# Yunwei729/WACV2023-High-Resolution-Depth-Estimation-for-Panoramas-Through-Perspective-Map-Registrations

Measured on AMD Instinct MI355X. Metric: panoramas/sec (whole node), 2048×1024 × 20 tiles, at 1/2/4/8 MI355X, higher is better.
Workload: dtype f32; 1 GPU; C3/C4: 64 panoramas per GPU per step, 2048x1024 output, 20 tiles of 512x512 (5x4 layout), 512x256 baseline; global_batch=64, out=2048x1024, tiles=20x512x512, parallelism=dp1 (panorama sharding, no collective)

## Files before the change

wacv2023-high-resolution-depth-estimation-for-panoramas-through-perspective-map-registrations_amd/csrc/pf_ctx.hpp:

```cpp
#pragma once
#include "../../include/panofuse.h"
#include "pf_internal.hpp"

#include <cstdarg>
#include <cstdio>
#include <cstring>
#include <string>
#include <vector>

namespace pf {

struct DevBuf {
    void* p = nullptr;
    size_t bytes = 0;
    DevBuf() = default;
    DevBuf(const DevBuf&) = delete;
    DevBuf& operator=(const DevBuf&) = delete;
    ~DevBuf()
    {
        if (p) (void)hipFree(p);
    }
};

struct LevelCache {
// ... 231 lines not shown

inline int check_tile_range(pf_ctx* c, int t0, int t1)
{
    if (t0 < 0 || t1 > c->ntiles || t0 > t1)
        return fail(c, PF_EINVAL, "tile range [%d,%d) outside [0,%d)", t0, t1, c->ntiles);
    return PF_OK;
}

int prepare_levels(pf_ctx* c, int out_w, int out_h, float zr0, float zr1);
int prepare_registration(pf_ctx* c, float zr0, float zr1);
const int2* reg_sample_index(pf_ctx* c, int ew, int eh, int ec);
const float* reg_sample_kf(pf_ctx* c, int ew, int eh, int ec);
int check_reg_grids(pf_ctx* c, const int* active);
void grid_tables(const LevelDims& L, std::vector<GridCol>& cols, std::vector<GridRow>& rows);

inline int level_at(pf_ctx* c, int out_w, int out_h, float zr0, float zr1, int level,
                    const LevelDims** L)
{
    int rc;
    if ((rc = prepare_levels(c, out_w, out_h, zr0, zr1))) return rc;
    if (level < 0 || level >= c->lc.nlevels) return fail(c, PF_EINVAL, "bad level %d", level);
    *L = &c->lc.dims[level];
    return PF_OK;
}

struct PassPlan {
    int T = 1, nchunks = 1;
    int stages = 1;
    double cost = 0;
};

struct JresPlan {
    bool on = false;
    int nb = 0, core = 0, K = 0, rounds = 0;
    bool half = false;
};

inline int strip_halo(int T) { return (T + kJacobiCols - 1) / kJacobiCols * kJacobiCols; }

struct StripGeom {
    int Tp, V, nstrips;
};
inline StripGeom strip_geometry(int T, int w)
{
    const int Tp = strip_halo(T), V = 64 * kJacobiCols - 2 * Tp;
    return {Tp, V, (w + V - 1) / V};
}

int jacobi_tcap(const LevelDims& L);
std::vector<PassPlan> plan_level(pf_ctx* c, const LevelDims& L, int tcap, int batch, bool fast,
                                 int band_rows = 0);
PassPlan plan_band_pass(pf_ctx* c, const LevelDims& L, int T, int band_rows, bool fast);
JresPlan jres_plan(pf_ctx* c, const LevelDims& L, int batch, bool fast);

struct JacobiRun {
    int first;
    const float* emap;
    int ew, eh, ec;
    long long estride;
    const GridCol* cols;
    const GridRow* rows;
    const float* prev;
    long long pstride;
    const float* lnorm;
    float *a, *b;
    uint16_t* out;
    long long ostride;
// ... 32 lines not shown
```

wacv2023-high-resolution-depth-estimation-for-panoramas-through-perspective-map-registrations_amd/csrc/pf_fuse.hip:

```cpp
#include "pf_ctx.hpp"

#include <cstdlib>

using namespace pf;

int pf::seed_tables(pf_ctx* c, const LevelDims& L, int ew, int eh, int ec)
{
    if (seed_tables_match(c, L, ew, eh, ec)) return PF_OK;
    std::vector<int> ecol(L.w + 2), erow(L.h + 2);
    for (int xx = -1; xx <= L.w; xx++) {
        const float az = (float)((double)((float)xx / (float)(L.w - 1) * 2.0f) * PF_MYPI);
        ecol[xx + 1] = (int)((double)az / (PF_MYPI * 2) * (double)(float)(ew - 1)) * ec;
    }
    for (int yy = -1; yy <= L.h; yy++) {
        const float zen = (float)((double)((float)yy / (float)(L.h - 1)) * PF_MYPI);
        erow[yy + 1] = (int)((double)zen / PF_MYPI * (double)(float)(eh - 1)) * ew * ec;
    }
    int rc;
    if ((rc = upload(c, c->seed_ecol, ecol)) || (rc = upload(c, c->seed_erow, erow))) return rc;
    const int key[5] = {L.w, L.h, ew, eh, ec};
    memcpy(c->seed_key, key, sizeof(key));
    return PF_OK;
}

// ... 36 lines not shown

static bool show_plans()
{
    static const bool show = getenv("PF_JPLAN") != nullptr;
    return show;
}

void pf::show_sweeps_plan(const LevelDims& L, int batch)
{
    if (show_plans())
        fprintf(stderr, "jacobi plan %dx%d band %d iters %d batch %d sweeps\n", L.w, L.h,
                L.h1 - L.h0 + 1, L.iters, batch);
}

static float* run_jres(pf_ctx* c, const LevelDims& L, const JacobiRun& r, const JresPlan& jp)
{
    JresArgs A{};
    A.src_mode = r.first;
    if (r.first == 2) {
        if (!r.emap || !seed_tables_match(c, L, r.ew, r.eh, r.ec)) return nullptr;
        A.ecol = (const int*)c->seed_ecol.p;
        A.erow = (const int*)c->seed_erow.p;
    }
    const long long st = (long long)L.w * L.h;
    A.src = r.a; A.sstride = st;
    A.prev = r.prev; A.pstride = r.pstride;
    A.emap = r.emap; A.estride = r.estride;
    A.lnorm = r.lnorm; A.lstride = st;
    A.hcol = r.hcol;
    float* dst = r.first == 0 ? r.b : r.a;
    A.dst = dst; A.dstride = st;
    A.out = r.out; A.ostride = r.ostride;
    A.w = L.w; A.h = L.h; A.h0 = L.h0; A.h1 = L.h1; A.iters = L.iters; A.batch = r.batch;
    A.nb = jp.nb; A.core = jp.core; A.K = jp.K; A.half = jp.half ? 1 : 0;
    uint32_t* sync = (uint32_t*)c->jres_sync.p;
    A.xbuf = (float*)c->jres_x.p;
    A.ticket = sync;
    A.err = sync + 1;
    A.flags = sync + 2;
    A.err_host = c->jres_err_h;
    static const int dbg = getenv("PF_JRES_DBG") ? atoi(getenv("PF_JRES_DBG")) : 0;
    A.dbg = dbg;
    A.spin_log2 = 24;
    if (c->jres_fault) {
        A.dbg |= 16;
        A.spin_log2 = c->jres_fault;
        c->jres_fault = 0;
    }
    A.tbase = c->jres_tk;
    A.fbase = c->jres_fb;
    c->jres_tk += (uint32_t)(r.batch * jp.nb);
    c->jres_fb += (uint32_t)(jp.rounds + 1);
    if (show_plans())
        fprintf(stderr, "jacobi plan %dx%d band %d iters %d batch %d resident: nb %d core %d K %d rounds %d\n",
                L.w, L.h, L.h1 - L.h0 + 1, L.iters, r.batch, jp.nb, jp.core, jp.K, jp.rounds);
    launch_jres(c->stream, A);
    return dst;
}

float* pf::run_jacobi(pf_ctx* c, const LevelDims& L, const JacobiRun& r, int* npasses)
{
    if (r.jp && r.jp->on) {
        if (npasses) *npasses = 1;
        return run_jres(c, L, r, *r.jp);
    }
    static const bool slow = getenv("PF_JSLOW") != nullptr;
    const bool fast = r.hcol && !slow;
    const std::vector<PassPlan> plan = plan_level(c, L, jacobi_tcap(L), r.batch, fast);
    if (r.first == 2 && r.emap && !seed_tables_match(c, L, r.ew, r.eh, r.ec)) return nullptr;
    JacobiPass P = jacobi_pass(c, L, r);
    const int band_rows = L.h1 - L.h0 + 1;
    float* src = (r.first == 0) ? r.a : nullptr;
    float* dst = (r.first == 0) ? r.b : r.a;
    if (show_plans()) {
        fprintf(stderr, "jacobi plan %dx%d band %d iters %d batch %d %s C%d:", L.w, L.h,
                band_rows, L.iters, r.batch, fast ? "packed" : "general", kJacobiCols);
        for (const PassPlan& pp : plan)
            fprintf(stderr, " T%d/n%d%s", pp.T, pp.nchunks, pp.stages > 1 ? "p" : "");
        fprintf(stderr, "\n");
    }
    int pass = 0;
    for (const PassPlan& pp : plan) {
        const int T = pp.T;
        set_pass_shape(P, T, band_rows, pp.nchunks);
        P.src_mode = pass == 0 ? r.first : 0;
        P.src = src;
        P.dst = dst;
        P.out_mode = (pass + 1 == (int)plan.size() && r.out) ? 1 : 0;
// ... 384 lines not shown
```

wacv2023-high-resolution-depth-estimation-for-panoramas-through-perspective-map-registrations_amd/csrc/pf_internal.hpp:

```cpp
#pragma once

#include <hip/hip_runtime.h>
#include <cstdint>
#include <vector>

#include "../../include/panofuse.h"

#pragma clang fp contract(off)

#define PF_MYPI 3.14159265359
#define PF_NAN_MARKER 0x7FBADBADu
#define PF_MAX_COVER 40

namespace pf {

struct TileGeom {
    float middle[3], hedge[3], vedge[3], corner0[3];
    float mm, hl, vl, pad;
    int w, h, c;
    int pix_off;
    long long off;
};

struct TileBox {
// ... 135 lines not shown
    int y = (int)((double)zen / PF_MYPI * (double)(float)(h - 1));
    return ((long long)y * w + x) * c;
}

static constexpr int kJacobiCols = 2;

struct JacobiPass {
    const float* src; long long sstride;
    const float* prev; long long pstride;
    const float* emap; long long estride;
    int ew, eh, ec, src_mode;
    const int* ecol; const int* erow;
    const GridCol* cols; const GridRow* rows;
    const float* lnorm; long long lstride;
    float* dst; long long dstride;
    uint16_t* out; long long ostride;
    int out_mode;
    int w, h, h0, h1;
    int V, Tp, nstrips, nchunks, rows_per_chunk;
    int row_lo, row_hi;
    const float* hcol;
};

struct JresArgs {
    const float* src; long long sstride;
    const float* prev; long long pstride;
    const float* emap; long long estride;
    const int* ecol; const int* erow;
    const float* lnorm; long long lstride;
    const float* hcol;
    float* dst; long long dstride;
    uint16_t* out; long long ostride;
    int w, h, h0, h1, iters, batch, src_mode;
    int nb, core, K;
    int half;
    float* xbuf;
    uint32_t* flags;
    uint32_t* ticket;
    uint32_t* err;
    uint32_t* err_host;
    uint32_t tbase, fbase;
    int dbg;
    int spin_log2;
};
int jres_region_rows(int w, bool half = false);
int jres_threads();
int jres_blocks_per_cu(int w, bool half);
void launch_jres(hipStream_t s, const JresArgs& A);

void launch_tapmap(hipStream_t s, const TileGeom* geom, const TapBox* tb, int ntiles,
                   long long max_points, const GridCol* cols, const GridRow* rows, int32_t* map);
static constexpr int kAuditWords = 6;
void launch_layout_audit(hipStream_t s, const TileGeom* geom, const TileBox* box, int ntiles,
                         const GridCol* cols, const GridRow* rows, LevelDims L,
                         unsigned long long* ctr);
void launch_targets_patch(hipStream_t s, const TileGeom* geom, const TileBox* box,
                          const TapBox* tb, int ntiles, const int32_t* map, const float* tiles,
                          long long tstride, const float* coeffs, LevelDims L, float* lnorm,
                          long long lstride, int batch, const uint32_t* tmask = nullptr,
                          int nmw = 0, TileValid tv = TileValid{0, 0.0f, 0.0f});
struct TgtLevel {
    LevelDims L;
    const TileBox* box;
    const uint32_t* tmask;
    int nmw;
    const TapBox* tb;
    const int32_t* map;
// ... 257 lines not shown
```

wacv2023-high-resolution-depth-estimation-for-panoramas-through-perspective-map-registrations_amd/csrc/pf_jacobi.hip:

```cpp
#include "pf_internal.hpp"

#include <cstdlib>
#include <cstring>

#ifndef PF_JLAG_WAVES
#define PF_JLAG_WAVES 1
#endif
#ifndef PF_JPK_GROUP
#define PF_JPK_GROUP 3
#endif
#ifndef PF_JFILL
#define PF_JFILL -1
#endif
#ifndef PF_JDRAIN
#define PF_JDRAIN 1
#endif
#ifndef PF_JLAG_WAVES_FAST
#define PF_JLAG_WAVES_FAST 3
#endif
#ifndef PF_JPIPE_FILL
#define PF_JPIPE_FILL 3
#endif
#ifndef PF_JLAG_PF
#define PF_JLAG_PF 2
#endif
static_assert(6 % (PF_JLAG_PF + 1) == 0, "the 6-step unroll needs a load-buffer period dividing 6");

namespace pf {

namespace {

__device__ __forceinline__ float dpp_from_left(float v)
{
    return __int_as_float(__builtin_amdgcn_mov_dpp(__float_as_int(v), 0x138, 0xF, 0xF, true));
}
__device__ __forceinline__ float dpp_from_right(float v)
{
    return __int_as_float(__builtin_amdgcn_mov_dpp(__float_as_int(v), 0x130, 0xF, 0xF, true));
}

typedef float f2 __attribute__((ext_vector_type(2)));

struct Row {
    f2 v;
};

}

enum { SRC_BUF = 0, SRC_UPSAMPLE = 1, SRC_SEED = 2 };

__device__ __forceinline__ f2 pk_add_clamp01(f2 a, f2 b)
{
    f2 r;
    asm("v_pk_add_f32 %0, %1, %2 clamp" : "=v"(r) : "v"(a), "v"(b));
    return r;
}

__device__ __forceinline__ float add_scalar(float a, float b)
{
    float r;
    asm("v_add_f32 %0, %1, %2" : "=v"(r) : "v"(a), "v"(b));
    return r;
}
__device__ __forceinline__ float fmac_from_right(float acc, float x, float q)
{
    asm("v_fmac_f32_dpp %0, %1, %2 wave_shl:1 row_mask:0xf bank_mask:0xf bound_ctrl:0"
        : "+v"(acc) : "v"(x), "v"(q));
    return acc;
}
__device__ __forceinline__ float fma_scalar(float a, float b, float c)
{
    float r;
    asm("v_fma_f32 %0, %1, %2, %3" : "=v"(r) : "v"(a), "v"(b), "v"(c));
    return r;
}

template <int T, int SRC, bool OUT16, bool FAST>
struct JLag {
    static constexpr int C = kJacobiCols;
    static_assert(C == 2, "a lane's columns are one pair: Row, the vector loads and stores, the wrap");
    static constexpr int PF = PF_JLAG_PF, NB = PF_JLAG_PF + 1;
    static constexpr int R = (2 * T + 1 + 5) / 6 * 6, NG = R / 6;
    Row Lr[R];
    Row H[T][3];
    Row In[NB];
    Row Lin[NB];
    float hcol[C];
    float vq;
    const JacobiPass* P;
    int w, xs0, vlo, vhi, r0, r1, h0, h1;
    int colbase;
    int lo;
    int rlo, rhi;
    const float *src, *prev, *emap, *lnorm;
    float* dst;
    uint16_t* out;

    __device__ __forceinline__ Row load_row(const float* base_ptr, int k) const
    {
        Row r;
        int kc = k < rlo ? rlo : (k > rhi ? rhi : k);
        const float* rp = base_ptr + ((long long)kc * w + colbase);
        float2 q = *reinterpret_cast<const float2*>(rp + lo);
        r.v[0] = q.x; r.v[1] = q.y;
        return r;
    }

    __device__ __forceinline__ Row load_input(int k) const
    {
        if constexpr (SRC == SRC_BUF) {
            return load_row(src, k);
        } else {
            Row r;
#pragma unroll
            for (int j = 0; j < C; j += 2) {
                int xr = xs0 + j, Y = k;
                if (xr < 0) { xr += w; Y -= 1; }
                else if (xr >= w) { xr -= w; Y += 1; }
                float v0 = 0.0f, v1 = 0.0f;
                if (Y >= 0 && Y < P->h) {
                    if constexpr (SRC == SRC_UPSAMPLE) {
                        v0 = v1 = prev[(long long)(Y >> 1) * (w >> 1) + (xr >> 1)];
                    } else if (Y >= P->h0 && Y <= P->h1) {
                        const int ro = P->erow[Y + 1];
                        v0 = emap[ro + P->ecol[xr + 1]];
                        v1 = emap[ro + P->ecol[xr + 2]];
                    }
                }
                r.v[j] = v0;
                r.v[j + 1] = v1;
            }
            return r;
        }
    }

    static constexpr int slot(int ph, int a) { return ((ph - a) % 3 + 3) % 3; }

    template <int GB, int PH>
    __device__ __forceinline__ void ring_put(Row r)
    {
        if constexpr (FAST) {
#pragma unroll
            for (int j = 0; j < C; j++) r.v[j] = __builtin_isfinite(r.v[j]) ? r.v[j] : 0.0f;
        }
        Lr[((GB + PH) % R + R) % R] = r;
// ... 107 lines not shown
            f2 hh = f2{hcol[0], hcol[1]};
            if constexpr (ROWS) {
                const int row = k - 2 * t;
                const float hr = (row == h0 || row == h1) ? 0.0f : 1.0f;
                hh = hh * hr;
            }
            cur[g] = __builtin_elementwise_fma(Lv[g].v - cur[g], hh, H[t - 1][slot(PH, 2 * t)].v);
        }
#pragma unroll
        for (int g = 0; g < G; g++) {
            const int t = T0 + 1 + g;
            nw[t - 1].v = pk_add_clamp01(cur[g] * reg_, H[t - 1][slot(PH, 2 * t)].v * reg);
        }
    }
    template <int PH, int GB, int T0, bool ROWS, int NA, int LA = 1>
    __device__ __forceinline__ void sweep_packed(Row* nw, int k) const
    {
        constexpr int T1 = T0 + PF_JPK_GROUP < T ? T0 + PF_JPK_GROUP : T;
        if constexpr (T1 < T) sweep_packed<PH, GB, T1, ROWS, NA, LA>(nw, k);
        constexpr int TB = T1 < NA ? T1 : NA;
        constexpr int TA = T0 > LA - 1 ? T0 : LA - 1;
        if constexpr (TA < TB) {
            Row Lv[TB - TA];
            ring_get_range<GB, PH, TA + 1, TB>(Lv);
            sweep_packed_group<PH, TA, TB, ROWS>(Lv, nw, k);
        }
    }

    template <int PH, bool ROWS, int GB, int NA = T, int LA = 1>
    __device__ __forceinline__ void step(int k)
    {
        H[0][slot(PH, 1)] = In[(PH + NB - 1) % NB];
        ring_put<GB, PH>(Lin[PH % NB]);
        Lin[(PH + PF) % NB] = load_row(lnorm, k + PF);
        In[(PH + PF - 1) % NB] = load_input(k + PF - 1);
        Row nw[T];
        if constexpr (FAST) {
            sweep_packed<PH, GB, 0, ROWS, NA, LA>(nw, k);
        } else {
            static_assert(NA == T && LA == 1, "the general form has no fill / drain specialisation");
            Row Lv[T];
            ring_get_range<GB, PH, 1, T>(Lv);
            sweep_general<PH>(Lv, nw);
        }
#pragma unroll
        for (int t = 1; t < T; t++)
            if (t >= LA && t <= NA) H[t][slot(PH, 2 * t)] = nw[t - 1];
        if constexpr (NA < T) return;
        const int j = k - 2 * T;
        if (j >= r0 && j < r1 && xs0 >= vlo && xs0 < vhi) {
            const long long rowb = (long long)j * w + colbase;
            if constexpr (OUT16) {
                uint32_t qv[C];
#pragma unroll
                for (int p = 0; p < C; p++) qv[p] = (uint32_t)(nw[T - 1].v[p] * 65535.0f);
                *reinterpret_cast<uint32_t*>(out + rowb + lo) = qv[0] | (qv[1] << 16);
            } else {
                *reinterpret_cast<float2*>(dst + rowb + lo) = make_float2(nw[T - 1].v[0], nw[T - 1].v[1]);
            }
        }
    }

    template <bool ROWS, int G>
    __device__ __forceinline__ void group(int k)
    {
        step<0, ROWS, 6 * G>(k);
        step<1, ROWS, 6 * G>(k + 1);
// ... 91 lines not shown
        const bool dr = ND > 0 && gt >= NF + ND;
        if (!fill_from<ROWS, 0>(k, kend)) return;
        const int kd = dr ? k0 + 6 * (gt - ND) : kend;
        if (k < kd) {
            bool more = true;
            if constexpr (NF % NG != 0) more = groups_from<ROWS, NF % NG>(k, kd);
            while (more) more = groups_from<ROWS, 0>(k, kd);
        }
        if (dr) drain<ROWS>(__builtin_amdgcn_readfirstlane((gt - ND) % NG), k);
    }
};

template <int T, int SRC, bool OUT16, bool FAST>
__global__ void __launch_bounds__(256, FAST ? PF_JLAG_WAVES_FAST : PF_JLAG_WAVES)
k_jlag(JacobiPass P)
{
    using S_t = JLag<T, SRC, OUT16, FAST>;
    constexpr int C = S_t::C;
    const int lane = threadIdx.x & 63;
    const int wave = __builtin_amdgcn_readfirstlane(threadIdx.x >> 6);
    const int job = blockIdx.x * 4 + wave;
    if (job >= P.nstrips * P.nchunks) return;
    const int b = blockIdx.y;
    const int strip = job % P.nstrips, chunk = job / P.nstrips;
    S_t S;
    S.P = &P;
    S.w = P.w;
    S.h0 = P.h0;
    S.h1 = P.h1;
    S.colbase = strip * P.V - P.Tp;
    S.lo = lane * C;
    S.vq = -0.25f;
    asm volatile("" : "+v"(S.vq));
    S.rlo = P.h0;
    S.rhi = P.h1;
    S.xs0 = strip * P.V - P.Tp + lane * C;
    S.vlo = strip * P.V;
    S.vhi = min(S.vlo + P.V, P.w);
    S.r0 = P.row_lo + chunk * P.rows_per_chunk;
    S.r1 = min(S.r0 + P.rows_per_chunk, P.row_hi);
    S.src = P.src + b * P.sstride;
    S.prev = P.prev + b * P.pstride;
    S.emap = P.emap + b * P.estride;
    S.lnorm = P.lnorm + b * P.lstride;
    S.dst = P.dst + b * P.dstride;
    S.out = P.out + b * P.ostride;
#pragma unroll
    for (int j = 0; j < C; j++) S.hcol[j] = 0.0f;
    if constexpr (FAST) {
        if (S.xs0 >= 0 && S.xs0 < P.w)
#pragma unroll
            for (int j = 0; j < C; j++) S.hcol[j] = P.hcol[S.xs0 + j];
    }
#pragma unroll
    for (int t = 0; t < T; t++)
#pragma unroll
        for (int q = 0; q < 3; q++)
#pragma unroll
            for (int j = 0; j < C; j++) S.H[t][q].v[j] = 0.0f;
#pragma unroll
    for (int q = 0; q < S_t::NB; q++)
#pragma unroll
        for (int j = 0; j < C; j++) { S.In[q].v[j] = 0.0f; S.Lin[q].v[j] = 0.0f; }
#pragma unroll
    for (int q = 0; q < S_t::R; q++)
#pragma unroll
        for (int j = 0; j < C; j++) S.Lr[q].v[j] = 0.0f;
    const int k0 = S.r0 - T - 1;
    const int kend = S.r1 + 2 * T;
#pragma unroll
    for (int r = 0; r + 1 < S_t::PF; r++) S.In[r] = S.load_input(k0 + r);
#pragma unroll
    for (int r = 0; r < S_t::PF; r++) S.Lin[r] = S.load_row(S.lnorm, k0 + r);
    const int wlo = k0 - 2 * T, whi = kend + 3;
    const bool rows = (S.h0 >= wlo && S.h0 <= whi) || (S.h1 >= wlo && S.h1 <= whi);
    if (!FAST || rows) S.template run<true>(k0, kend);
    else S.template run<false>(k0, kend);
}

static constexpr int md(int a, int m) { return ((a % m) + m) % m; }

template <int TS, int S, int SI, int SRC, bool OUT16>
struct JPipe {
    static constexpr int C = kJacobiCols;
    static constexpr int T = TS * S;
    static constexpr int TB = SI * TS + 1, TE = TB + TS - 1;
    static constexpr int PF = PF_JLAG_PF, NB = PF_JLAG_PF + 1;
    static constexpr int R = (2 * TS + 1 + 5) / 6 * 6;
    static constexpr int NG = R / 6;
    static constexpr int G = PF_JPK_GROUP;
    Row H[TS][3];
    Row In[NB];
    Row Lin[NB];
    float* lring;
    const float* xin;
    float* xout;
    int lane_c;
    float hcol[C];
    float vq;
    const JacobiPass* P;
    int w, xs0, vlo, vhi, r0, r1, h0, h1, colbase, lo, rlo, rhi;
    const float *src, *prev, *emap, *lnorm;
    float* dst;
    uint16_t* out;

    __device__ __forceinline__ Row load_row(const float* base_ptr, int k) const
    {
        Row r;
        int kc = k < rlo ? rlo : (k > rhi ? rhi : k);
        const float2 q = *reinterpret_cast<const float2*>(base_ptr + ((long long)kc * w + colbase) + lo);
        r.v[0] = q.x; r.v[1] = q.y;
        return r;
    }
    __device__ __forceinline__ Row load_input(int k) const
    {
        if constexpr (SRC == SRC_BUF) {
            return load_row(src, k);
        } else {
            Row r;
            int xr = xs0, Y = k;
            if (xr < 0) { xr += w; Y -= 1; }
            else if (xr >= w) { xr -= w; Y += 1; }
            float v0 = 0.0f, v1 = 0.0f;
            if (Y >= 0 && Y < P->h) {
                if constexpr (SRC == SRC_UPSAMPLE) {
                    v0 = v1 = prev[(long long)(Y >> 1) * (w >> 1) + (xr >> 1)];
                } else if (Y >= P->h0 && Y <= P->h1) {
                    const int ro = P->erow[Y + 1];
                    v0 = emap[ro + P->ecol[xr + 1]];
                    v1 = emap[ro + P->ecol[xr + 2]];
                }
            }
            r.v[0] = v0;
            r.v[1] = v1;
            return r;
        }
    }
    __device__ __forceinline__ void lds_put(float* p, Row r) const
    {
        r.v[0] = __builtin_isfinite(r.v[0]) ? r.v[0] : 0.0f;
        r.v[1] = __builtin_isfinite(r.v[1]) ? r.v[1] : 0.0f;
        *reinterpret_cast<float2*>(p) = make_float2(r.v[0], r.v[1]);
    }
    __device__ __forceinline__ Row lds_get(const float* p) const
    {
        Row r;
        const float2 q = *reinterpret_cast<const float2*>(p);
        r.v[0] = q.x; r.v[1] = q.y;
        return r;
    }

    template <int PH, int T0, int T1, bool ROWS>
// ... 37 lines not shown
                const float hr = (row == h0 || row == h1) ? 0.0f : 1.0f;
                hh = hh * hr;
            }
            cur[g] = __builtin_elementwise_fma(Lv[t - TB].v - cur[g], hh, H[l][md(PH - 2 * t, 3)].v);
        }
#pragma unroll
        for (int g = 0; g < NGR; g++) {
            const int t = T0 + 1 + g, l = t - TB;
            nw[t - TB].v = pk_add_clamp01(cur[g] * reg_, H[l][md(PH - 2 * t, 3)].v * reg);
        }
    }
    template <int PH, int T0, bool ROWS, int NA>
    __device__ __forceinline__ void sweep(const Row* Lv, Row* nw, int k) const
    {
        constexpr int T1 = T0 + G < TE ? T0 + G : TE;
        constexpr int TB_ = T1 < NA ? T1 : NA;
        if constexpr (T0 < TB_) sweep_group<PH, T0, TB_, ROWS>(Lv, nw, k);
        if constexpr (T1 < TE) sweep<PH, T1, ROWS, NA>(Lv, nw, k);
    }

    template <int PH, bool ROWS, int GB, int NA = T>
    __device__ __forceinline__ void step(int k)
    {
        if constexpr (SI == 0) {
            H[0][md(PH - 1, 3)] = In[md(PH - 1, NB)];
        } else {
            H[0][md(PH - 2 * TB + 1, 3)] = lds_get(xin + md(PH - 1, 2) * (64 * C) + lane_c);
        }
        constexpr int QO = -2 * TB + 2;
        lds_put(lring + md(GB + PH + QO, R) * (64 * C) + lane_c, Lin[md(PH + QO, NB)]);
        Row Lv[TS];
#pragma unroll
        for (int t = TB; t <= TE; t++) Lv[t - TB] = lds_get(lring + md(GB + PH - 2 * t, R) * (64 * C) + lane_c);
        Lin[md(PH + QO + PF, NB)] = load_row(lnorm, k + QO + PF);
        if constexpr (SI == 0) In[md(PH + PF - 1, NB)] = load_input(k + PF - 1);
        Row nw[TS];
        sweep<PH, TB - 1, ROWS, NA>(Lv, nw, k);
#pragma unroll
        for (int t = TB; t < TE; t++)
            if (t <= NA) H[t - TB + 1][md(PH - 2 * t, 3)] = nw[t - TB];
        if constexpr (SI < S - 1) {
            if constexpr (TE <= NA)
                *reinterpret_cast<float2*>(xout + md(PH, 2) * (64 * C) + lane_c) =
                    make_float2(nw[TS - 1].v[0], nw[TS - 1].v[1]);
        } else if constexpr (NA == T) {
            const int j = k - 2 * T;
            if (j >= r0 && j < r1 && xs0 >= vlo && xs0 < vhi) {
                const long long rowb = (long long)j * w + colbase;
                if constexpr (OUT16) {
                    const uint32_t q0 = (uint32_t)(nw[TS - 1].v[0] * 65535.0f);
                    const uint32_t q1 = (uint32_t)(nw[TS - 1].v[1] * 65535.0f);
                    *reinterpret_cast<uint32_t*>(out + rowb + lo) = q0 | (q1 << 16);
                } else {
                    *reinterpret_cast<float2*>(dst + rowb + lo) =
                        make_float2(nw[TS - 1].v[0], nw[TS - 1].v[1]);
                }
            }
        }
        __syncthreads();
    }

    template <bool ROWS, int GI>
    __device__ __forceinline__ void group(int k)
    {
        step<0, ROWS, 6 * GI>(k);
        step<1, ROWS, 6 * GI>(k + 1);
        step<2, ROWS, 6 * GI>(k + 2);
// ... 34 lines not shown
            return fill_from<ROWS, F + 1>(k, kend);
        } else {
            return true;
        }
    }
    template <bool ROWS>
    __device__ __forceinline__ void run(int k0, int kend)
    {
        int k = k0;
        bool more = fill_from<ROWS, 0>(k, kend);
        if constexpr (NF % NG != 0) {
            if (more) more = groups_from<ROWS, NF % NG>(k, kend);
        }
        while (more) more = groups_from<ROWS, 0>(k, kend);
    }
};

template <int TS, int S, int SI, int SRC, bool OUT16>
__device__ __forceinline__ void jpipe_stage(const JacobiPass& P, int lane, int b, int strip,
                                            int chunk, float* lring, float* xchg)
{
    using S_t = JPipe<TS, S, SI, SRC, OUT16>;
    constexpr int T = S_t::T, C = S_t::C;
    S_t St;
    St.P = &P;
    St.w = P.w;
    St.h0 = P.h0;
    St.h1 = P.h1;
    St.colbase = strip * P.V - P.Tp;
    St.lo = lane * C;
    St.lane_c = lane * C;
    St.vq = -0.25f;
    asm volatile("" : "+v"(St.vq));
    St.rlo = P.h0;
    St.rhi = P.h1;
    St.xs0 = strip * P.V - P.Tp + lane * C;
    St.vlo = strip * P.V;
    St.vhi = min(St.vlo + P.V, P.w);
    St.r0 = P.row_lo + chunk * P.rows_per_chunk;
    St.r1 = min(St.r0 + P.rows_per_chunk, P.row_hi);
    St.src = P.src + b * P.sstride;
    St.prev = P.prev + b * P.pstride;
    St.emap = P.emap + b * P.estride;
    St.lnorm = P.lnorm + b * P.lstride;
    St.dst = P.dst + b * P.dstride;
    St.out = P.out + b * P.ostride;
    St.lring = lring + SI * (S_t::R * 64 * C);
    St.xin = SI > 0 ? xchg + (SI - 1) * (2 * 64 * C) : nullptr;
    St.xout = SI < S - 1 ? xchg + SI * (2 * 64 * C) : nullptr;
    St.hcol[0] = St.hcol[1] = 0.0f;
    if (St.xs0 >= 0 && St.xs0 < P.w) { St.hcol[0] = P.hcol[St.xs0]; St.hcol[1] = P.hcol[St.xs0 + 1]; }
#pragma unroll
    for (int l = 0; l < TS; l++)
#pragma unroll
        for (int q = 0; q < 3; q++) St.H[l][q].v = f2{0.0f, 0.0f};
#pragma unroll
    for (int q = 0; q < S_t::NB; q++) { St.In[q].v = f2{0.0f, 0.0f}; St.Lin[q].v = f2{0.0f, 0.0f}; }
    const int k0 = St.r0 - T - 1;
    const int kend = St.r1 + 2 * T;
    constexpr int QO = -2 * S_t::TB + 2;
    if constexpr (SI == 0) {
#pragma unroll
        for (int r = 0; r + 1 < S_t::PF; r++) St.In[md(r, S_t::NB)] = St.load_input(k0 + r);
    }
#pragma unroll
    for (int r = 0; r < S_t::PF; r++) St.Lin[md(QO + r, S_t::NB)] = St.load_row(St.lnorm, k0 + QO + r);
    const int wlo = k0 - 2 * T, whi = kend + 3;
    const bool rows = (St.h0 >= wlo && St.h0 <= whi) || (St.h1 >= wlo && St.h1 <= whi);
    if (rows) St.template run<true>(k0, kend);
    else St.template run<false>(k0, kend);
}

template <int TS, int S, int SRC, bool OUT16>
__global__ void __launch_bounds__(64 * S) k_jpipe(JacobiPass P)
{
    constexpr int C = kJacobiCols, R = JPipe<TS, S, 0, SRC, OUT16>::R;
    const int lane = threadIdx.x & 63;
    const int wave = __builtin_amdgcn_readfirstlane(threadIdx.x >> 6);
    const int job = blockIdx.x;
    if (job >= P.nstrips * P.nchunks) return;
    const int b = blockIdx.y;
    const int strip = job % P.nstrips, chunk = job / P.nstrips;
    __shared__ float lring[S * R * 64 * C];
    __shared__ float xchg[(S > 1 ? S - 1 : 1) * 2 * 64 * C];
    for (int i = threadIdx.x; i < (S > 1 ? S - 1 : 1) * 2 * 64 * C; i += 64 * S) xchg[i] = 0.0f;
    __syncthreads();
    if (wave == 0) jpipe_stage<TS, S, 0, SRC, OUT16>(P, lane, b, strip, chunk, lring, xchg);
    if constexpr (S > 1) { if (wave == 1) jpipe_stage<TS, S, (S > 1 ? 1 : 0), SRC, OUT16>(P, lane, b, strip, chunk, lring, xchg); }
    if constexpr (S > 2) { if (wave == 2) jpipe_stage<TS, S, (S > 2 ? 2 : 0), SRC, OUT16>(P, lane, b, strip, chunk, lring, xchg); }
    if constexpr (S > 3) { if (wave == 3) jpipe_stage<TS, S, (S > 3 ? 3 : 0), SRC, OUT16>(P, lane, b, strip, chunk, lring, xchg); }
}

#if !defined(PF_JPART) || PF_JPART == 0
__global__ void __launch_bounds__(256) k_border(const float* __restrict__ prev, long long pstride,
                                                LevelDims L, float* __restrict__ a,
                                                float* __restrict__ bb, long long stride,
                                                uint16_t* __restrict__ out, long long ostride)
{
    const int top = L.h0 * L.w;
// ... 214 lines not shown
```

wacv2023-high-resolution-depth-estimation-for-panoramas-through-perspective-map-registrations_amd/csrc/pf_jres.hip:

```cpp
#include "pf_internal.hpp"

namespace pf {

namespace {

typedef float f2 __attribute__((ext_vector_type(2)));
typedef uint32_t u4v __attribute__((ext_vector_type(4)));

__device__ __forceinline__ float dpp_shr(float v)
{
    return __int_as_float(__builtin_amdgcn_mov_dpp(__float_as_int(v), 0x138, 0xF, 0xF, true));
}
__device__ __forceinline__ float dpp_rol(float v)
{
    return __int_as_float(__builtin_amdgcn_mov_dpp(__float_as_int(v), 0x134, 0xF, 0xF, false));
}
__device__ __forceinline__ float fmac_rol(float acc, float x, float q)
{
    asm("s_nop 1\n\tv_fmac_f32_dpp %0, %1, %2 wave_rol:1 row_mask:0xf bank_mask:0xf"
        : "+v"(acc) : "v"(x), "v"(q));
    return acc;
}
__device__ __forceinline__ f2 pk_add_clamp01(f2 a, f2 b)
{
// ... 91 lines not shown
        f2 up[NP], dn[NP], s1[NP], n[NP];
#pragma unroll
        for (int k = 0; k < NP; k++) {
            up[k] = up_lds ? up_lds[64 * k] : f2{0.0f, 0.0f};
            dn[k] = dn_lds ? dn_lds[64 * k] : f2{0.0f, 0.0f};
            s1[k] = b[RS > 1 ? 1 : 0][k];
            n[k] = b[0][k];
        }
        if constexpr (RS > 1) rows_mid<1, HAS_EDGE>(n, dn, em);
        if (HAS_EDGE && (em & 1u)) row<0, true>(up, RS > 1 ? s1 : dn);
        else row<0, false>(up, RS > 1 ? s1 : dn);
    }
};

template <int CPL, int RS, int NWV, int SRC, bool OUT16>
__global__ void __launch_bounds__(64 * NWV) k_jres(JresArgs A)
{
    using S_t = JRes<CPL, RS, NWV, SRC, OUT16>;
    constexpr int NP = S_t::NP, NW = S_t::NW;
    __shared__ f2 lds_edge[2][2][NW][NP][64];
    __shared__ uint32_t lds_ticket;
    const int tid = threadIdx.x;
    S_t S;
    S.lane = tid & 63;
    S.wv = __builtin_amdgcn_readfirstlane(tid >> 6);
    S.vq = -0.25f;
    asm volatile("" : "+v"(S.vq));
    const int lane = S.lane, wv = S.wv;
    if (tid == 0) lds_ticket = __hip_atomic_fetch_add(A.ticket, 1u, __ATOMIC_RELAXED, __HIP_MEMORY_SCOPE_AGENT);
    __syncthreads();
    const uint32_t t = __builtin_amdgcn_readfirstlane(lds_ticket - A.tbase);
    const int p = (int)(t / (uint32_t)A.nb), j = (int)(t % (uint32_t)A.nb);
    const int w = A.w;
    const int c0 = A.h0 + j * A.core;
    const int c1 = min(c0 + A.core, A.h1 + 1);
    const int K = A.K;
    const int rs = j == 0 ? A.h0 : c0 - K;
    const int re = j == A.nb - 1 ? A.h1 + 1 : min(c1 + K, A.h1 + 1);
    const int x0 = lane * CPL;
    const int qc0 = c0 - rs, qc1 = c1 - rs;

    {
        const float* lp = A.lnorm + p * A.lstride;
#pragma unroll
        for (int k = 0; k < NP; k++) {
            S.hc[k].x = A.hcol[x0 + 2 * k];
            S.hc[k].y = A.hcol[x0 + 2 * k + 1];
        }
#pragma unroll
        for (int r = 0; r < RS; r++) {
            const int Y = rs + wv * RS + r;
            const bool live = Y < re;
#pragma unroll
            for (int k = 0; k < NP; k++) {
                float v0 = 0.0f, v1 = 0.0f, l0 = 0.0f, l1 = 0.0f;
                if (live) {
                    const int x = x0 + 2 * k;
                    if constexpr (SRC == 2) {
                        const float* ep = A.emap + p * A.estride + A.erow[Y + 1];
                        v0 = ep[A.ecol[x + 1]];
                        v1 = ep[A.ecol[x + 2]];
                    } else if constexpr (SRC == 1) {
                        v0 = v1 = A.prev[p * A.pstride + (long long)(Y >> 1) * (w >> 1) + (x >> 1)];
                    } else {
                        const float2 q = *reinterpret_cast<const float2*>(A.src + p * A.sstride + (long long)Y * w + x);
                        v0 = q.x;
                        v1 = q.y;
                    }
// ... 211 lines not shown
```

wacv2023-high-resolution-depth-estimation-for-panoramas-through-perspective-map-registrations_amd/csrc/pf_plan.hip:

```cpp
#include "pf_ctx.hpp"

#include <cstdlib>

using namespace pf;

static int plan_simds(const pf_ctx* c)
{
    const int n = (int)(4.0 * c->num_cu * c->jacobi_share + 0.5);
    return n < 4 ? 4 : n;
}

struct JacobiTuning {
    int Tmax = 10;
    double step_overhead = 3.0, lone_cycles = 4.0;
    double pipe_overhead = 1.0;
    double launch_cost = 300.0;
};

static const JacobiTuning& jacobi_tuning()
{
    static const JacobiTuning tune = [] {
        JacobiTuning t;
        if (const char* e = getenv("PF_JT")) t.Tmax = atoi(e);
        if (const char* e = getenv("PF_JOVH")) t.step_overhead = atof(e);
// ... 81 lines not shown
    for (int r = L.iters; r > 0; r -= choice[r]) plan.push_back(opt[choice[r]]);
    if (c->jacobi_share < 1.0)
        for (PassPlan& pp : plan)
            if (pp.stages == 1)
                pp.nchunks = best_chunks(pp.T, band_rows, L.w, batch,
                                         jstream_waves_per_cu(pp.T, fast) / 4, plan_simds(c))
                                 .nchunks;
    char key[32];
    snprintf(key, sizeof(key), "PF_JN%d", L.w);
    if (const char* e = getenv(key))
        for (PassPlan& pp : plan) pp.nchunks = atoi(e) > 0 ? atoi(e) : pp.nchunks;
    return plan;
}

int pf::jacobi_tcap(const LevelDims& L)
{
    int cap = jacobi_tuning().Tmax;
    char key[32];
    snprintf(key, sizeof(key), "PF_JT%d", L.w);
    if (const char* e = getenv(key)) cap = atoi(e) > 0 ? atoi(e) : cap;
    if (L.h0 - 1 < cap) cap = L.h0 - 1;
    if (L.h - 2 - L.h1 < cap) cap = L.h - 2 - L.h1;
    while (cap >= 1) {
        int Tp = (cap + 3) / 4 * 4;
        if (128 - Tp <= L.w && L.w % 2 == 0) break;
        cap--;
    }
    return cap;
}

PassPlan pf::plan_band_pass(pf_ctx* c, const LevelDims& L, int T, int band_rows, bool fast)
{
    return best_chunks(T, band_rows, L.w, 1, jstream_waves_per_cu(T, fast) / 4, plan_simds(c));
}

JresPlan pf::jres_plan(pf_ctx* c, const LevelDims& L, int batch, bool fast)
{
    JresPlan jp;
    static const char* env = getenv("PF_JRES");
    const int mode = c->jres_mode >= 0 ? c->jres_mode : (env && atoi(env) == 0 ? 0 : 1);
    if (mode == 0 || !fast || batch < 1) return jp;
    const int rows = jres_region_rows(L.w);
    if (rows <= 0 || L.iters < 1) return jp;
    static int bpc_w[2][2] = {{-1, -1}, {-1, -1}};
    const int wi = L.w == 256 ? 0 : 1;
    const int band = L.h1 - L.h0 + 1;
    static const double xcost = getenv("PF_JRES_X") ? atof(getenv("PF_JRES_X")) : 2.5;
    static const int nb_env = getenv("PF_JRES_NB") ? atoi(getenv("PF_JRES_NB")) : 0;
    const int nb_force = c->jres_nb > 0 ? c->jres_nb : nb_env;
    static const double hcost = getenv("PF_JRES_HALFCOST") ? atof(getenv("PF_JRES_HALFCOST")) : 0.6;
    double best = 1e300;
    for (int hv = 0; hv < 2; hv++) {
        const int rows_h = hv ? jres_region_rows(L.w, true) : rows;
        if (rows_h <= 0) continue;
        if (bpc_w[wi][hv] < 0) bpc_w[wi][hv] = jres_blocks_per_cu(L.w, hv == 1);
        const int bpc = bpc_w[wi][hv];
        if (bpc < 1) continue;
        const double sweep = hv ? hcost : 1.0;
        for (int nb = 1; nb <= band && nb <= 64; nb++) {
            if (nb_force > 0 && nb != nb_force) continue;
            const int core = (band + nb - 1) / nb;
            if ((band + core - 1) / core != nb) continue;
            int K;
            if (nb == 1) {
                if (core > rows_h) continue;
                K = L.iters;
            } else {
                K = (rows_h - core) / 2;
                if (K > core) K = core;
                if (K > L.iters) K = L.iters;
                if (K < 1) continue;
            }
            const int rounds = (L.iters + K - 1) / K;
            const long long resident = (long long)c->num_cu * bpc;
            const long long waves = ((long long)batch * nb + resident - 1) / resident;
            const double cost = (double)waves * (L.iters * sweep + (rounds - 1) * xcost);
            if (cost < best) {
                best = cost;
                jp.on = true;
                jp.nb = nb;
                jp.core = core;
                jp.K = K;
                jp.rounds = rounds;
                jp.half = hv == 1;
            }
        }
    }
    return jp;
}
```

Baseline: 18160 panoramas/s.

## Use asymmetric edge/interior block cores in resident Jacobi and tighten row clamp windows

The resident Jacobi planner now lets edge blocks own a larger core (rows minus one halo) than interior blocks (rows minus two halos). It picks K from the register-resident row capacity, which should allow a larger K and fewer exchange rounds for the same block count. The streaming Jacobi kernels also clamp input and lnorm row loads to a per-chunk window widened by the halo rather than the whole band, which limits out-of-window reads. Risks are off-by-one errors in the block bounds and in the clamping, which could change numerics at chunk edges.

```diff
diff --git a/wacv2023-high-resolution-depth-estimation-for-panoramas-through-perspective-map-registrations_amd/csrc/pf_ctx.hpp b/wacv2023-high-resolution-depth-estimation-for-panoramas-through-perspective-map-registrations_amd/csrc/pf_ctx.hpp
--- a/wacv2023-high-resolution-depth-estimation-for-panoramas-through-perspective-map-registrations_amd/csrc/pf_ctx.hpp
+++ b/wacv2023-high-resolution-depth-estimation-for-panoramas-through-perspective-map-registrations_amd/csrc/pf_ctx.hpp
@@ -287,7 +287,7 @@
 
 struct JresPlan {
     bool on = false;
-    int nb = 0, core = 0, K = 0, rounds = 0;
+    int nb = 0, core_e = 0, core_i = 0, K = 0, rounds = 0;
     bool half = false;
 };
 
diff --git a/wacv2023-high-resolution-depth-estimation-for-panoramas-through-perspective-map-registrations_amd/csrc/pf_fuse.hip b/wacv2023-high-resolution-depth-estimation-for-panoramas-through-perspective-map-registrations_amd/csrc/pf_fuse.hip
--- a/wacv2023-high-resolution-depth-estimation-for-panoramas-through-perspective-map-registrations_amd/csrc/pf_fuse.hip
+++ b/wacv2023-high-resolution-depth-estimation-for-panoramas-through-perspective-map-registrations_amd/csrc/pf_fuse.hip
@@ -92,7 +92,7 @@
     A.dst = dst; A.dstride = st;
     A.out = r.out; A.ostride = r.ostride;
     A.w = L.w; A.h = L.h; A.h0 = L.h0; A.h1 = L.h1; A.iters = L.iters; A.batch = r.batch;
-    A.nb = jp.nb; A.core = jp.core; A.K = jp.K; A.half = jp.half ? 1 : 0;
+    A.nb = jp.nb; A.core_e = jp.core_e; A.core_i = jp.core_i; A.K = jp.K; A.half = jp.half ? 1 : 0;
     uint32_t* sync = (uint32_t*)c->jres_sync.p;
     A.xbuf = (float*)c->jres_x.p;
     A.ticket = sync;
@@ -112,8 +112,9 @@
     c->jres_tk += (uint32_t)(r.batch * jp.nb);
     c->jres_fb += (uint32_t)(jp.rounds + 1);
     if (show_plans())
-        fprintf(stderr, "jacobi plan %dx%d band %d iters %d batch %d resident: nb %d core %d K %d rounds %d\n",
-                L.w, L.h, L.h1 - L.h0 + 1, L.iters, r.batch, jp.nb, jp.core, jp.K, jp.rounds);
+        fprintf(stderr, "jacobi plan %dx%d band %d iters %d batch %d resident: nb %d core %d/%d K %d rounds %d\n",
+                L.w, L.h, L.h1 - L.h0 + 1, L.iters, r.batch, jp.nb, jp.core_e, jp.core_i, jp.K,
+                jp.rounds);
     launch_jres(c->stream, A);
     return dst;
 }
diff --git a/wacv2023-high-resolution-depth-estimation-for-panoramas-through-perspective-map-registrations_amd/csrc/pf_internal.hpp b/wacv2023-high-resolution-depth-estimation-for-panoramas-through-perspective-map-registrations_amd/csrc/pf_internal.hpp
--- a/wacv2023-high-resolution-depth-estimation-for-panoramas-through-perspective-map-registrations_amd/csrc/pf_internal.hpp
+++ b/wacv2023-high-resolution-depth-estimation-for-panoramas-through-perspective-map-registrations_amd/csrc/pf_internal.hpp
@@ -191,7 +191,7 @@
     float* dst; long long dstride;
     uint16_t* out; long long ostride;
     int w, h, h0, h1, iters, batch, src_mode;
-    int nb, core, K;
+    int nb, core_e, core_i, K;
     int half;
     float* xbuf;
     uint32_t* flags;
diff --git a/wacv2023-high-resolution-depth-estimation-for-panoramas-through-perspective-map-registrations_amd/csrc/pf_jacobi.hip b/wacv2023-high-resolution-depth-estimation-for-panoramas-through-perspective-map-registrations_amd/csrc/pf_jacobi.hip
--- a/wacv2023-high-resolution-depth-estimation-for-panoramas-through-perspective-map-registrations_amd/csrc/pf_jacobi.hip
+++ b/wacv2023-high-resolution-depth-estimation-for-panoramas-through-perspective-map-registrations_amd/csrc/pf_jacobi.hip
@@ -45,6 +45,12 @@
     f2 v;
 };
 
+__device__ __forceinline__ void row_window(int r0, int r1, int d, int h0, int h1, int& lo, int& hi)
+{
+    lo = min(max(r0 - d, h0), h1);
+    hi = max(min(r1 + d - 1, h1), lo);
+}
+
 }
 
 enum { SRC_BUF = 0, SRC_UPSAMPLE = 1, SRC_SEED = 2 };
@@ -91,12 +97,12 @@
     int w, xs0, vlo, vhi, r0, r1, h0, h1;
     int colbase;
     int lo;
-    int rlo, rhi;
+    int ilo, ihi, llo, lhi;
     const float *src, *prev, *emap, *lnorm;
     float* dst;
     uint16_t* out;
 
-    __device__ __forceinline__ Row load_row(const float* base_ptr, int k) const
+    __device__ __forceinline__ Row load_row(const float* base_ptr, int k, int rlo, int rhi) const
     {
         Row r;
         int kc = k < rlo ? rlo : (k > rhi ? rhi : k);
@@ -109,8 +115,9 @@
     __device__ __forceinline__ Row load_input(int k) const
     {
         if constexpr (SRC == SRC_BUF) {
-            return load_row(src, k);
+            return load_row(src, k, ilo, ihi);
         } else {
+            k = k < ilo ? ilo : (k > ihi ? ihi : k);
             Row r;
 #pragma unroll
             for (int j = 0; j < C; j += 2) {
@@ -284,7 +291,7 @@
     {
         H[0][slot(PH, 1)] = In[(PH + NB - 1) % NB];
         ring_put<GB, PH>(Lin[PH % NB]);
-        Lin[(PH + PF) % NB] = load_row(lnorm, k + PF);
+        Lin[(PH + PF) % NB] = load_row(lnorm, k + PF, llo, lhi);
         In[(PH + PF - 1) % NB] = load_input(k + PF - 1);
         Row nw[T];
         if constexpr (FAST) {
@@ -442,13 +449,13 @@
     S.lo = lane * C;
     S.vq = -0.25f;
     asm volatile("" : "+v"(S.vq));
-    S.rlo = P.h0;
-    S.rhi = P.h1;
     S.xs0 = strip * P.V - P.Tp + lane * C;
     S.vlo = strip * P.V;
     S.vhi = min(S.vlo + P.V, P.w);
     S.r0 = P.row_lo + chunk * P.rows_per_chunk;
     S.r1 = min(S.r0 + P.rows_per_chunk, P.row_hi);
+    row_window(S.r0, S.r1, T, P.h0, P.h1, S.ilo, S.ihi);
+    row_window(S.r0, S.r1, T - 1, P.h0, P.h1, S.llo, S.lhi);
     S.src = P.src + b * P.sstride;
     S.prev = P.prev + b * P.pstride;
     S.emap = P.emap + b * P.estride;
@@ -481,7 +488,7 @@
 #pragma unroll
     for (int r = 0; r + 1 < S_t::PF; r++) S.In[r] = S.load_input(k0 + r);
 #pragma unroll
-    for (int r = 0; r < S_t::PF; r++) S.Lin[r] = S.load_row(S.lnorm, k0 + r);
+    for (int r = 0; r < S_t::PF; r++) S.Lin[r] = S.load_row(S.lnorm, k0 + r, S.llo, S.lhi);
     const int wlo = k0 - 2 * T, whi = kend + 3;
     const bool rows = (S.h0 >= wlo && S.h0 <= whi) || (S.h1 >= wlo && S.h1 <= whi);
     if (!FAST || rows) S.template run<true>(k0, kend);
@@ -509,12 +516,13 @@
     float hcol[C];
     float vq;
     const JacobiPass* P;
-    int w, xs0, vlo, vhi, r0, r1, h0, h1, colbase, lo, rlo, rhi;
+    int w, xs0, vlo, vhi, r0, r1, h0, h1, colbase, lo;
+    int ilo, ihi, llo, lhi;
     const float *src, *prev, *emap, *lnorm;
     float* dst;
     uint16_t* out;
 
-    __device__ __forceinline__ Row load_row(const float* base_ptr, int k) const
+    __device__ __forceinline__ Row load_row(const float* base_ptr, int k, int rlo, int rhi) const
     {
         Row r;
         int kc = k < rlo ? rlo : (k > rhi ? rhi : k);
@@ -525,9 +533,10 @@
     __device__ __forceinline__ Row load_input(int k) const
     {
         if constexpr (SRC == SRC_BUF) {
-            return load_row(src, k);
+            return load_row(src, k, ilo, ihi);
         } else {
             Row r;
+            k = k < ilo ? ilo : (k > ihi ? ihi : k);
             int xr = xs0, Y = k;
             if (xr < 0) { xr += w; Y -= 1; }
             else if (xr >= w) { xr -= w; Y += 1; }
@@ -631,7 +640,7 @@
         Row Lv[TS];
 #pragma unroll
         for (int t = TB; t <= TE; t++) Lv[t - TB] = lds_get(lring + md(GB + PH - 2 * t, R) * (64 * C) + lane_c);
-        Lin[md(PH + QO + PF, NB)] = load_row(lnorm, k + QO + PF);
+        Lin[md(PH + QO + PF, NB)] = load_row(lnorm, k + QO + PF, llo, lhi);
         if constexpr (SI == 0) In[md(PH + PF - 1, NB)] = load_input(k + PF - 1);
         Row nw[TS];
         sweep<PH, TB - 1, ROWS, NA>(Lv, nw, k);
@@ -732,13 +741,13 @@
     St.lane_c = lane * C;
     St.vq = -0.25f;
     asm volatile("" : "+v"(St.vq));
-    St.rlo = P.h0;
-    St.rhi = P.h1;
     St.xs0 = strip * P.V - P.Tp + lane * C;
     St.vlo = strip * P.V;
     St.vhi = min(St.vlo + P.V, P.w);
     St.r0 = P.row_lo + chunk * P.rows_per_chunk;
     St.r1 = min(St.r0 + P.rows_per_chunk, P.row_hi);
+    row_window(St.r0, St.r1, T, P.h0, P.h1, St.ilo, St.ihi);
+    row_window(St.r0, St.r1, T - S_t::TB, P.h0, P.h1, St.llo, St.lhi);
     St.src = P.src + b * P.sstride;
     St.prev = P.prev + b * P.pstride;
     St.emap = P.emap + b * P.estride;
@@ -764,7 +773,7 @@
         for (int r = 0; r + 1 < S_t::PF; r++) St.In[md(r, S_t::NB)] = St.load_input(k0 + r);
     }
 #pragma unroll
-    for (int r = 0; r < S_t::PF; r++) St.Lin[md(QO + r, S_t::NB)] = St.load_row(St.lnorm, k0 + QO + r);
+    for (int r = 0; r < S_t::PF; r++) St.Lin[md(QO + r, S_t::NB)] = St.load_row(St.lnorm, k0 + QO + r, St.llo, St.lhi);
     const int wlo = k0 - 2 * T, whi = kend + 3;
     const bool rows = (St.h0 >= wlo && St.h0 <= whi) || (St.h1 >= wlo && St.h1 <= whi);
     if (rows) St.template run<true>(k0, kend);
diff --git a/wacv2023-high-resolution-depth-estimation-for-panoramas-through-perspective-map-registrations_amd/csrc/pf_jres.hip b/wacv2023-high-resolution-depth-estimation-for-panoramas-through-perspective-map-registrations_amd/csrc/pf_jres.hip
--- a/wacv2023-high-resolution-depth-estimation-for-panoramas-through-perspective-map-registrations_amd/csrc/pf_jres.hip
+++ b/wacv2023-high-resolution-depth-estimation-for-panoramas-through-perspective-map-registrations_amd/csrc/pf_jres.hip
@@ -147,8 +147,8 @@
     const uint32_t t = __builtin_amdgcn_readfirstlane(lds_ticket - A.tbase);
     const int p = (int)(t / (uint32_t)A.nb), j = (int)(t % (uint32_t)A.nb);
     const int w = A.w;
-    const int c0 = A.h0 + j * A.core;
-    const int c1 = min(c0 + A.core, A.h1 + 1);
+    const int c0 = A.h0 + (j == 0 ? 0 : A.core_e + (j - 1) * A.core_i);
+    const int c1 = min(c0 + (j == 0 || j == A.nb - 1 ? A.core_e : A.core_i), A.h1 + 1);
     const int K = A.K;
     const int rs = j == 0 ? A.h0 : c0 - K;
     const int re = j == A.nb - 1 ? A.h1 + 1 : min(c1 + K, A.h1 + 1);
diff --git a/wacv2023-high-resolution-depth-estimation-for-panoramas-through-perspective-map-registrations_amd/csrc/pf_plan.hip b/wacv2023-high-resolution-depth-estimation-for-panoramas-through-perspective-map-registrations_amd/csrc/pf_plan.hip
--- a/wacv2023-high-resolution-depth-estimation-for-panoramas-through-perspective-map-registrations_amd/csrc/pf_plan.hip
+++ b/wacv2023-high-resolution-depth-estimation-for-panoramas-through-perspective-map-registrations_amd/csrc/pf_plan.hip
@@ -137,6 +137,27 @@
 PassPlan pf::plan_band_pass(pf_ctx* c, const LevelDims& L, int T, int band_rows, bool fast)
 {
     return best_chunks(T, band_rows, L.w, 1, jstream_waves_per_cu(T, fast) / 4, plan_simds(c));
+}
+
+static bool jres_blocking(int band, int nb, int rows, int iters, int& core_e, int& core_i, int& K)
+{
+    K = (nb * rows - band) / (2 * nb - 2);
+    const int kcap = nb > 2 ? rows / 3 : rows / 2;
+    if (K > kcap) K = kcap;
+    if (K > iters) K = iters;
+    if (K >= 1) {
+        core_e = rows - K;
+        core_i = rows - 2 * K;
+        const int last = band - core_e - (nb - 2) * core_i;
+        if (last >= 1 && last <= core_e) return true;
+    }
+    const int core = (band + nb - 1) / nb;
+    if ((band + core - 1) / core != nb) return false;
+    K = (rows - core) / 2;
+    if (K > core) K = core;
+    if (K > iters) K = iters;
+    core_e = core_i = core;
+    return K >= 1;
 }
 
 JresPlan pf::jres_plan(pf_ctx* c, const LevelDims& L, int batch, bool fast)
@@ -164,17 +185,11 @@
         const double sweep = hv ? hcost : 1.0;
         for (int nb = 1; nb <= band && nb <= 64; nb++) {
             if (nb_force > 0 && nb != nb_force) continue;
-            const int core = (band + nb - 1) / nb;
-            if ((band + core - 1) / core != nb) continue;
-            int K;
+            int core_e = band, core_i = band, K = L.iters;
             if (nb == 1) {
-                if (core > rows_h) continue;
-                K = L.iters;
-            } else {
-                K = (rows_h - core) / 2;
-                if (K > core) K = core;
-                if (K > L.iters) K = L.iters;
-                if (K < 1) continue;
+                if (band > rows_h) continue;
+            } else if (!jres_blocking(band, nb, rows_h, L.iters, core_e, core_i, K)) {
+                continue;
             }
             const int rounds = (L.iters + K - 1) / K;
             const long long resident = (long long)c->num_cu * bpc;
@@ -184,7 +199,8 @@
                 best = cost;
                 jp.on = true;
                 jp.nb = nb;
-                jp.core = core;
+                jp.core_e = core_e;
+                jp.core_i = core_i;
                 jp.K = K;
                 jp.rounds = rounds;
                 jp.half = hv == 1;
```

Measured after the change: 18320 panoramas/s (median of 6 runs). About the same (+0.9%).
